# LFY1998/IPDM-PyTorch

Hardware: AMD Instinct MI355X
Metric: CT slices/s (full proj+img partial-diffusion sample) (higher is better)
Workload: dtype f32

## Files before the change

### include/ipdm_hip.h

```cpp
#ifndef IPDM_HIP_H
#define IPDM_HIP_H
#include <stddef.h>
#include <stdint.h>

#ifdef __cplusplus
extern "C" {
#endif

#define IPDM_OK 0
#define IPDM_ERR_INVALID (-1)
#define IPDM_ERR_HIP (-2)
#define IPDM_ERR_WORKSPACE (-3)
#define IPDM_ERR_UNSUPPORTED (-4)

const char *ipdm_last_error(void);
#define IPDM_ABI_VERSION 5
int ipdm_abi_version(void);

int ipdm_set_option(const char *name, int value);
int ipdm_get_option(const char *name, int *value);

typedef struct ipdm_fbp_geom {
    int32_t n_views, n_det, grid_n;
    double da, det_offset, dtheta_deg, source_origin, fov_half;
// ... 142 lines not shown
int ipdm_metrics_plan_destroy(ipdm_metrics_plan *plan);
size_t ipdm_metrics_workspace_bytes(const ipdm_metrics_plan *plan, int32_t B, uint32_t mask);
int ipdm_metrics(ipdm_metrics_plan *plan, const float *d_ref, int64_t ref_stride, const float *d_img, int32_t B,
                 uint32_t mask, double *d_out, void *d_ws, size_t ws_bytes, void *stream);
int64_t ipdm_metrics_table(const ipdm_metrics_plan *plan, int32_t which, void *host_out, int64_t cap_elems);

int ipdm_lowdose_noise(const float *d_proj, const float *d_z1, const float *d_z2, float *d_out, int32_t B,
                       int64_t n_per_slice, double factor, double n0, double ne, int32_t model, void *stream);
int ipdm_lowdose_noise_rng(const float *d_proj, float *d_out, int32_t B, int64_t n_per_slice, double factor, double n0,
                           double ne, int32_t model, uint64_t seed, int64_t slice_id0, int64_t draw0, void *stream);

#define IPDM_PROF_CLASSES 8
int ipdm_profile_begin(int32_t max_launches);
int ipdm_profile_begin_classes(int32_t max_launches, uint32_t class_mask);
int ipdm_profile_end(double *out_flops, double *out_ms, int64_t *out_launches, int32_t n_classes);
int ipdm_clock_probe(uint64_t *d_out, int32_t samples, int32_t period_us, void *stream);

int ipdm_bench_conv2d(int32_t B, int32_t C1, int32_t C2, int32_t H, int32_t W, int32_t Cout, int32_t ksize,
                      int32_t stride, int32_t act, int32_t with_res, int32_t iters, float *avg_ms);
int ipdm_bench_attention(int32_t B, int32_t heads, int32_t d, int32_t T, int32_t iters, float *avg_ms);
int32_t ipdm_conv_layout_code(int32_t Cout, int32_t ksize, int32_t stride);
int32_t ipdm_conv_kernel_code(int32_t B, int32_t Cout, int32_t Cin, int32_t ksize, int32_t stride, int32_t H, int32_t W);
int32_t ipdm_conv_kernel_code_stats(int32_t B, int32_t Cout, int32_t Cin, int32_t ksize, int32_t stride, int32_t H, int32_t W);
int32_t ipdm_attention_kernel_code(int32_t d);

#ifdef __cplusplus
}
#endif
#endif
```

### ipdm-pytorch_amd/_lib.py

```python
import ctypes as C
import os

_HERE = os.path.dirname(os.path.abspath(__file__))
LIB_PATH = os.environ.get("IPDM_LIB_PATH") or os.path.join(_HERE, "libipdm_hip.so")


class IpdmError(RuntimeError):
    pass


class FbpGeom(C.Structure):
    _fields_ = [("n_views", C.c_int32), ("n_det", C.c_int32), ("grid_n", C.c_int32),
                ("da", C.c_double), ("det_offset", C.c_double), ("dtheta_deg", C.c_double),
                ("source_origin", C.c_double), ("fov_half", C.c_double)]


class UnetCfg(C.Structure):
    _fields_ = [("in_channels", C.c_int32), ("model_channels", C.c_int32), ("out_channels", C.c_int32),
                ("num_res_blocks", C.c_int32), ("num_heads", C.c_int32), ("n_mult", C.c_int32),
                ("n_attn", C.c_int32), ("channel_mult", C.c_double * 16),
                ("attention_resolutions", C.c_int32 * 16)]


class ReverseArgs(C.Structure):
# ... 54 lines not shown
    "ipdm_ddpm_step_rng": (C.c_int, [_vp, _i32, _vp, _vp, _vp, _u64, _i64, _i64, _vp, _i32, _i32, _i32, _f64, _vp, _i32, _i32,
                                     _i32, _vp, _sz, _vp]),
    "ipdm_reverse_workspace_bytes": (_sz, [_vp, _i32, _i32, _i32]),
    "ipdm_reverse_pass": (C.c_int, [_vp, _vp, _vp, _vp, _vp, _i32, _i32, _vp, _i32, _i32, _i32, _i32, C.POINTER(ReverseArgs),
                                    _vp, _sz, _vp]),
    "ipdm_guided_reverse": (C.c_int, [_vp, _vp, _vp, _vp, _i32, _i32, _i32, C.POINTER(_i32), _i32, C.POINTER(ReverseArgs),
                                      C.POINTER(_i64), _vp, _sz, _vp]),
    "ipdm_op_conv2d": (C.c_int, [_vp, _i32, _vp, _i32, _i32, _i32, _i32, _i32, _i32, _vp, _vp, _i32, _i32, _i32,
                                 _i32, _i32, _vp, _vp, _vp, _vp, _vp]),
    "ipdm_op_conv_gn_conv": (C.c_int, [_vp, _i32, _i32, _i32, _i32, _vp, _vp, _i32, _i32, _i32, _vp, _i32, _vp, _vp, _i32, _vp, _vp,
                                       _i32, _vp, _vp, C.POINTER(_i32), _vp]),
    "ipdm_op_up_conv_chain": (C.c_int, [_vp, _i32, _i32, _i32, _i32, _vp, _vp, _i32, _vp, _i32, _i32, _vp, _vp, _i32, _vp, _vp,
                                        _i32, _i32, _vp, _vp, C.POINTER(_i32), _vp]),
    "ipdm_profile_begin": (C.c_int, [_i32]),
    "ipdm_profile_begin_classes": (C.c_int, [_i32, C.c_uint32]),
    "ipdm_clock_probe": (C.c_int, [_vp, _i32, _i32, _vp]),
    "ipdm_profile_end": (C.c_int, [C.POINTER(_f64 * PROF_CLASSES), C.POINTER(_f64 * PROF_CLASSES), C.POINTER(_i64 * PROF_CLASSES), _i32]),
    "ipdm_bench_conv2d": (C.c_int, [_i32] * 11 + [C.POINTER(_f32)]),
    "ipdm_bench_attention": (C.c_int, [_i32] * 5 + [C.POINTER(_f32)]),
    "ipdm_op_attention": (C.c_int, [_vp, _vp, _i32, _i32, _i32, _i32, _vp]),
    "ipdm_conv_layout_code": (_i32, [_i32, _i32, _i32]),
    "ipdm_conv_kernel_code": (_i32, [_i32, _i32, _i32, _i32, _i32, _i32, _i32]),
    "ipdm_conv_kernel_code_stats": (_i32, [_i32, _i32, _i32, _i32, _i32, _i32, _i32]),
    "ipdm_attention_kernel_code": (_i32, [_i32]),
    "ipdm_art_plan_create": (C.c_int, [_vp, _vp, _vp, C.POINTER(_vp)]),
    "ipdm_art_plan_destroy": (C.c_int, [_vp]),
    "ipdm_art_workspace_bytes": (C.c_size_t, [_vp, _i32]),
    "ipdm_art_reconstruct": (C.c_int, [_vp, _vp, _vp, _i32, _i32, _i32, _i32, _vp, C.c_size_t, _vp]),
    "ipdm_art_project": (C.c_int, [_vp, _vp, _vp, _i32, _vp, C.c_size_t, _vp]),
    "ipdm_metrics_plan_create": (C.c_int, [_i32, _i32, C.POINTER(_vp)]),
    "ipdm_metrics_plan_destroy": (C.c_int, [_vp]),
    "ipdm_metrics_workspace_bytes": (_sz, [_vp, _i32, C.c_uint32]),
    "ipdm_metrics": (C.c_int, [_vp, _vp, _i64, _vp, _i32, C.c_uint32, _vp, _vp, _sz, _vp]),
    "ipdm_metrics_table": (_i64, [_vp, _i32, _vp, _i64]),
    "ipdm_lowdose_noise": (C.c_int, [_vp, _vp, _vp, _vp, _i32, _i64, _f64, _f64, _f64, _i32, _vp]),
    "ipdm_lowdose_noise_rng": (C.c_int, [_vp, _vp, _i32, _i64, _f64, _f64, _f64, _i32, _u64, _i64, _i64, _vp]),
}

_lib = None


def lib():
    global _lib
    if _lib is None:
        if not os.path.isfile(LIB_PATH):
            raise IpdmError("%s not found: the HIP extension is mandatory (no CPU fallback). "
# ... 64 lines not shown
```

### ipdm-pytorch_amd/csrc/common.h

```cpp
#pragma once
#include <hip/hip_runtime.h>
#include <cstdarg>
#include <cstdio>
#include <cstring>
#include <string>
#include <vector>
#include "../../include/ipdm_hip.h"

namespace ipdm {

void set_error(const char *fmt, ...);

#define IPDM_HIP_CHECK(expr)                                                                   \
    do {                                                                                       \
        hipError_t e_ = (expr);                                                                \
        if (e_ != hipSuccess) {                                                                \
            ipdm::set_error("%s failed: %s (%s:%d)", #expr, hipGetErrorString(e_), __FILE__,  \
                            __LINE__);                                                         \
            return IPDM_ERR_HIP;                                                               \
        }                                                                                      \
    } while (0)

#define IPDM_REQUIRE(cond, ...)                   \
    do {                                          \
// ... 2 lines not shown
            return IPDM_ERR_INVALID;              \
        }                                         \
    } while (0)

#define IPDM_LAUNCH_CHECK() IPDM_HIP_CHECK(hipGetLastError())

static inline int cdiv(long a, long b) { return (int)((a + b - 1) / b); }
static inline size_t align_up(size_t v, size_t a) { return (v + a - 1) / a * a; }

enum Opt {
    OPT_CONV_NO_UP2,
    OPT_CONV_NO_WUP2,
    OPT_CONV_LEGACY, OPT_CONV1X1_LEGACY, OPT_CONVS2_LEGACY,
    OPT_CONV_NO_DIRECT, OPT_DIRECT_NO_PLANAR, OPT_DIRECT_MAX_CIN, OPT_DIRECT_NO_S2, OPT_DIRECT_NO_SKIP_FUSE,
    OPT_CONV_DBG, OPT_CONV_VEC4_STRICT, OPT_CONV_NO_SPLITK, OPT_CONV_NO_WINO, OPT_WINO_V1, OPT_WINO2_MIN_TILES, OPT_CONV1X1_NO_QUARTER, OPT_CONV_NO_PW, OPT_PW_ITEM, OPT_PW_FORCE,
    OPT_CONV_NM,
    OPT_GN_TWO_STAGE, OPT_GN_UNFUSED,
    OPT_UNET_TRANSPOSE,
    OPT_ATTN_NO_KVSPLIT, OPT_ATTN_LEGACY, OPT_ATTN_NO_ZSEQ,
    OPT_ART_PER_VIEW,
    OPT_CONV_BF16X3,
    OPT_ATTN_EXACT_F32,
    OPT_ATTN_NO_PRESPLIT,
    OPT_COUNT
};
int opt(Opt o);
bool opt_per_call(int o);
const char *opt_name(int o);
void opt_snapshot(int (&dst)[OPT_COUNT]);
int opt_changed_since(const int (&rec)[OPT_COUNT]);
std::vector<int> opt_per_call_values();

int ensure_dynamic_lds(const void *kernel, size_t bytes);
int device_cu_count();

int unet_io_channels(const ipdm_unet *net, int *cin, int *cout);

__device__ inline double wave_sum(double v)
{
#pragma unroll
    for (int o = 32; o > 0; o >>= 1) v += __shfl_down(v, o, 64);
    return v;
}
__device__ inline float wave_sum(float v)
{
#pragma unroll
// ... 12 lines not shown
```

### ipdm-pytorch_amd/csrc/common.hip

```cpp
#include <cctype>
#include <cstdlib>
#include <mutex>
#include <strings.h>
#include <set>
#include <utility>
#include "common.h"

namespace ipdm {
static thread_local char g_err[512] = "";
void set_error(const char *fmt, ...)
{
    va_list ap;
    va_start(ap, fmt);
    vsnprintf(g_err, sizeof(g_err), fmt, ap);
    va_end(ap);
}

namespace {
std::mutex g_attr_mu;
std::set<std::pair<const void *, int>> g_attr_done;
int g_cus[64];
}

namespace {
struct OptDef { const char *name; int def; bool per_call; int lo = 0, hi = 1; };
const OptDef g_opt_def[OPT_COUNT] = {
    {"conv_no_up2", 0, true},
    {"conv_no_wup2", 0, true},
    {"conv_legacy", 0, false}, {"conv1x1_legacy", 0, false}, {"convs2_legacy", 0, false},
    {"conv_no_direct", 0, false}, {"direct_no_planar", 0, false},
    {"direct_max_cin", 160, false, 0, 160},
    {"direct_no_s2", 0, false}, {"direct_no_skip_fuse", 0, true},
    {"conv_dbg", 0, true, 0, 0x3ff}, {"conv_vec4_strict", 0, false}, {"conv_no_splitk", 0, false},
    {"conv_no_wino", 0, true}, {"wino_v1", 0, true}, {"wino2_min_tiles", 192, true, 0, 1 << 24},
    {"conv1x1_no_quarter", 0, true}, {"conv_no_pw", 0, true}, {"pw_item", 0, true, 0, 2}, {"pw_force", 0, true}, {"conv_nm", 0, true, 0, 2},
    {"gn_two_stage", 0, true}, {"gn_unfused", 0, true},
    {"unet_transpose", -1, true, -1, 1},
    {"attn_no_kvsplit", 0, false}, {"attn_legacy", 0, false}, {"attn_no_zseq", 0, true},
    {"art_per_view", 0, true},
    {"conv_bf16x3", 0, true},
    {"attn_exact_f32", 0, true},
    {"attn_no_presplit", 0, true},
};
bool opt_value_ok(int i, int v)
{
    return v >= g_opt_def[i].lo && v <= g_opt_def[i].hi;
}
std::mutex g_opt_mu;
int g_opt_val[OPT_COUNT];
bool g_opt_init = false;

void opt_init_locked()
{
    if (g_opt_init) return;
    for (int i = 0; i < OPT_COUNT; ++i) {
        char env[64] = "IPDM_";
        size_t n = 5;
        for (const char *c = g_opt_def[i].name; *c && n + 1 < sizeof(env); ++c) env[n++] = (char)toupper((unsigned char)*c);
        env[n] = 0;
        const char *e = getenv(env);
        g_opt_val[i] = g_opt_def[i].def;
        if (e) {
            char *end = nullptr;
            const long v = strtol(e, &end, 10);
            const int want = (end != e) ? (int)v : 1;
// ... 93 lines not shown
```

### ipdm-pytorch_amd/csrc/conv_direct.hip

```cpp
#include <cstdlib>
#include <type_traits>
#include "common.h"
#include "unet_kernels.h"

using namespace ipdm;

typedef float f32x2 __attribute__((ext_vector_type(2)));
typedef float f32x4 __attribute__((ext_vector_type(4)));

namespace {

inline double direct_bytes(const ConvArgs &a)
{
    return 4.0 * a.B * ((double)(a.C1 + a.C2 + (a.sk_w ? a.sk_C1 + a.sk_C2 : 0)) * a.Hs * a.Ws + (double)a.Cout * a.Ho * a.Wo * (a.res ? 2 : 1));
}

inline bool direct_compute_bound(const ConvArgs &a) { return a.C1 + a.C2 >= 64; }
inline double direct_flops(const ConvArgs &a, int taps)
{
    return 2.0 * a.B * a.Ho * a.Wo * a.Cout * ((double)(a.C1 + a.C2) * taps + (a.sk_w ? a.sk_C1 + a.sk_C2 : 0));
}
inline int direct_class(const ConvArgs &a) { return direct_compute_bound(a) ? 6 : 4; }
inline double direct_work(const ConvArgs &a, int taps) { return direct_compute_bound(a) ? direct_flops(a, taps) : direct_bytes(a); }

// ... 12 lines not shown
    const int rest = t / gx;
    d.by = rest % gy;
    d.n = rest / gy;
    return d;
}
constexpr int DIN_P1 = 68;

#define IPDM_DPP_F(v, ctrl) __builtin_bit_cast(float, __builtin_amdgcn_update_dpp(0, __builtin_bit_cast(int, (v)), (ctrl), 0xf, 0xf, false))
__device__ inline float sum_lanes_row(float x)
{
    x += IPDM_DPP_F(x, 0x121);
    x += IPDM_DPP_F(x, 0x122);
    x += IPDM_DPP_F(x, 0x124);
    x += IPDM_DPP_F(x, 0x128);
    return x;
}
#undef IPDM_DPP_F

constexpr int DOOB = 0x7fffffff;
__device__ inline float dload(__amdgpu_buffer_rsrc_t r, int voff, int soff)
{
    return __builtin_bit_cast(float, __builtin_amdgcn_raw_buffer_load_b32(r, voff, soff, 0));
}

template <int CO>
__device__ inline void direct_epilogue(const ConvArgs &a, f32x2 (&acc)[4][CO / 2], int n, int ox0, int oy0, int tx, int ty, float *in_lds)
{
    const int tid = threadIdx.x;
    const int oy = oy0 + ty, ox = ox0 + tx * 4;
    const bool in_img = oy < a.Ho && ox < a.Wo;
    const size_t out_plane = (size_t)a.Ho * a.Wo;
    const bool vec = (a.Wo & 3) == 0;
    const bool full_tile = oy0 + DT_H <= a.Ho && ox0 + DT_W <= a.Wo;
    float *st = in_lds;
    if (a.stats) __syncthreads();
#pragma unroll
    for (int co = 0; co < CO; ++co) {
        if (co < a.Cout) {
            const float b = a.bias ? a.bias[co] : 0.0f;
            const size_t o = ((size_t)n * a.Cout + co) * out_plane + (size_t)oy * a.Wo + ox;
            f32x4 v = {acc[0][co / 2][co & 1] + b, acc[1][co / 2][co & 1] + b, acc[2][co / 2][co & 1] + b, acc[3][co / 2][co & 1] + b};
            if (in_img) {
                if (vec) {
                    if (a.res) v += *reinterpret_cast<const f32x4 *>(a.res + o);
                    *reinterpret_cast<f32x4 *>(a.out + o) = v;
                } else {
// ... 15 lines not shown
            }
        }
    }
    if (a.stats) {
        __syncthreads();
        const int j = tid & 15;
#pragma unroll
        for (int k = tid >> 4; k < 2 * CO; k += 16) {
            if ((k >> 1) < a.Cout) {
                const f32x4 *src = reinterpret_cast<const f32x4 *>(st + k * 256 + j * 16);
                const f32x4 p0 = src[0], p1 = src[1], p2 = src[2], p3 = src[3];
                float s = (((p0[0] + p0[1]) + (p0[2] + p0[3])) + ((p1[0] + p1[1]) + (p1[2] + p1[3]))) +
                          (((p2[0] + p2[1]) + (p2[2] + p2[3])) + ((p3[0] + p3[1]) + (p3[2] + p3[3])));
                s = sum_lanes_row(s);
                if (j == 0) {
                    const int row = (oy0 / DT_H) * gridDim.x + ox0 / DT_W;
                    a.stats[(((size_t)n * a.stats_rows + row) * a.Cout + (k >> 1)) * 2 + (k & 1)] = s;
                }
            }
        }
    }
}

template <int CO, int KS, int DKC, bool PLANAR, int STRIDE = 1, int SKIP = 0>
__global__ void __launch_bounds__(256, (STRIDE == 2 ? (CO <= 8 ? 4 : 3) : (CO <= 4 ? 6 : (CO <= 8 ? 5 : 3)))) conv_direct_kernel(ConvArgs a)
{
    static_assert(SKIP == 0 || (KS == 3 && STRIDE == 1 && !PLANAR), "conv_direct: the fused shortcut rides on a 3x3 stride-1 NCHW layer");
    constexpr int DIN_H = (DT_H - 1) * STRIDE + KS, DIN_W = (DT_W - 1) * STRIDE + KS, DIN_P = STRIDE == 1 ? DIN_P1 : 132;
    constexpr int DIN_CH = DIN_H * DIN_P, TAPS = KS * KS, PAD = KS / 2;
    static_assert(STRIDE == 1 || (KS == 3 && !PLANAR), "conv_direct: stride 2 is the 3x3 Downsample");
    __shared__ __attribute__((aligned(16))) float in_lds[DKC * DIN_CH];
    typedef const __attribute__((address_space(4))) float cfloat;
    cfloat *wk = (cfloat *)(unsigned long long)a.w;
    cfloat *gsc = (cfloat *)(unsigned long long)a.gn_scale, *gsh = (cfloat *)(unsigned long long)a.gn_shift;
    const int tid = threadIdx.x;
    const int tx = tid & 15, ty = tid >> 4;
    const DTile dt = direct_tile();
    const int n = dt.n;
    const int ox0 = dt.bx * DT_W, oy0 = dt.by * DT_H;
    const int Ctot = a.C1 + a.C2;
    const int src_plane = a.Hs * a.Ws;

    f32x2 acc[4][CO / 2];
#pragma unroll
    for (int p = 0; p < 4; ++p)
#pragma unroll
        for (int c = 0; c < CO / 2; ++c) acc[p][c] = f32x2{0.0f, 0.0f};

    constexpr int NSP = (DIN_H * DIN_W + 255) / 256;
    int sp_src[NSP], sp_srcp[NSP], sp_dst[NSP];
    bool sp_ok[NSP];
#pragma unroll
    for (int j = 0; j < NSP; ++j) {
        const int e = tid + j * 256;
        const int r = e / DIN_W, c = e % DIN_W;
        const int iy = oy0 * STRIDE - PAD + r, ix = ox0 * STRIDE - PAD + c;
        sp_ok[j] = e < DIN_H * DIN_W && iy >= 0 && iy < a.H && ix >= 0 && ix < a.W;
        int sy = min(max(iy, 0), a.H - 1), sx = min(max(ix, 0), a.W - 1);
        if (a.upsample) {
            sy = min((int)floorf((float)sy * a.scale_y), a.Hs - 1);
            sx = min((int)floorf((float)sx * a.scale_x), a.Ws - 1);
        }
        sp_src[j] = e < DIN_H * DIN_W ? (sy * a.Ws + sx) * 4 : DOOB;
        sp_srcp[j] = !(PLANAR || SKIP == 2) ? sp_src[j]
                   : (e < DIN_H * DIN_W ? ((((sy & 1) * 2 + (sx & 1)) * (a.Hs >> 1) + (sy >> 1)) * (a.Ws >> 1) + (sx >> 1)) * 4 : DOOB);
        sp_dst[j] = e < DIN_H * DIN_W ? r * DIN_P + c : -1;
    }
    const int plane_bytes = src_plane * 4;
    const __amdgpu_buffer_rsrc_t rsrc1 = __builtin_amdgcn_make_buffer_rsrc((void *)(a.x1 + (size_t)n * a.C1 * src_plane), 0, a.C1 * plane_bytes, 0x00020000);
    const __amdgpu_buffer_rsrc_t rsrc2 = __builtin_amdgcn_make_buffer_rsrc((void *)(a.x2 ? a.x2 + (size_t)n * a.C2 * src_plane : a.x1), 0, a.x2 ? a.C2 * plane_bytes : 0, 0x00020000);

    auto run_chunks = [&](auto sk_tag) __attribute__((always_inline)) {
    constexpr bool SK = decltype(sk_tag)::value;
    const int C1v = SK ? a.sk_C1 : a.C1, Ctotv = SK ? a.sk_C1 + a.sk_C2 : Ctot;
    const int actv = SK ? 0 : a.act;
    const __amdgpu_buffer_rsrc_t rsA = SK ? __builtin_amdgcn_make_buffer_rsrc((void *)(a.sk_x1 + (size_t)n * a.sk_C1 * src_plane), 0, a.sk_C1 * plane_bytes, 0x00020000) : rsrc1;
    const __amdgpu_buffer_rsrc_t rsB = SK ? __builtin_amdgcn_make_buffer_rsrc((void *)(a.sk_x2 ? a.sk_x2 + (size_t)n * a.sk_C2 * src_plane : a.sk_x1), 0,
                                                                               a.sk_x2 ? a.sk_C2 * plane_bytes : 0, 0x00020000) : rsrc2;
    constexpr bool PL = SK ? SKIP == 2 : PLANAR;
    cfloat *wkv = SK ? (cfloat *)(unsigned long long)a.sk_w : wk;
    const int cpadv = SK ? a.sk_cout_pad : a.cout_pad;
    for (int c0 = 0; c0 < Ctotv; c0 += DKC) {
        const int kc = min(DKC, Ctotv - c0);
        __syncthreads();
        float raw[DKC][NSP];
#pragma unroll
        for (int c = 0; c < DKC; ++c) {
            const int cg = min(c0 + c, Ctotv - 1);
            const bool from1 = cg < C1v;
            const __amdgpu_buffer_rsrc_t r = from1 ? rsA : rsB;
            const int so = (from1 ? cg : cg - C1v) * plane_bytes;
#pragma unroll
            for (int j = 0; j < NSP; ++j) raw[c][j] = dload(r, PL && from1 ? sp_srcp[j] : sp_src[j], so);
        }
#pragma unroll
        for (int c = 0; c < DKC; ++c) {
            if (c < kc) {
                float sc = 1.0f, sh = 0.0f;
                if (actv) { sc = gsc[(size_t)n * Ctot + c0 + c]; sh = gsh[(size_t)n * Ctot + c0 + c]; }
#pragma unroll
                for (int j = 0; j < NSP; ++j) {
                    float v = raw[c][j];
                    if (actv) {
                        v = v * sc + sh;
                        if (actv == 2) v = v * __builtin_amdgcn_rcpf(1.0f + __builtin_amdgcn_exp2f(-1.4426950408889634f * v));
                    }
                    if (sp_dst[j] >= 0) in_lds[c * DIN_CH + sp_dst[j]] = sp_ok[j] ? v : 0.0f;
                }
            }
        }
        __syncthreads();
        for (int c = 0; c < kc; ++c) {
            const float *ip = in_lds + c * DIN_CH + ty * STRIDE * DIN_P + tx * 4 * STRIDE;
#pragma unroll
            for (int ky = 0; ky < KS; ++ky) {
                if (SK && ky != 1) continue;
                const f32x4 lo = *reinterpret_cast<const f32x4 *>(ip + ky * DIN_P);
                f32x2 hi = {0.0f, 0.0f};
                if (KS > 1 && STRIDE == 1) hi = *reinterpret_cast<const f32x2 *>(ip + ky * DIN_P + 4);
                f32x4 mid = {0.0f, 0.0f, 0.0f, 0.0f};
                float last = 0.0f;
                if (STRIDE == 2) { mid = *reinterpret_cast<const f32x4 *>(ip + ky * DIN_P + 4); last = ip[ky * DIN_P + 8]; }
                const float iv[9] = {lo[0], lo[1], lo[2], lo[3], STRIDE == 1 ? hi[0] : mid[0], STRIDE == 1 ? hi[1] : mid[1], mid[2], mid[3], last};
#pragma unroll
                for (int kx = 0; kx < KS; ++kx) {
                    if (SK && kx != 1) continue;
                    cfloat *wp = wkv + (SK ? (size_t)(c0 + c) : (size_t)(c0 + c) * TAPS + ky * KS + kx) * cpadv;
                    f32x2 wv[CO / 2];
#pragma unroll
                    for (int q = 0; q < CO / 2; ++q) wv[q] = f32x2{wp[2 * q], wp[2 * q + 1]};
#pragma unroll
                    for (int p = 0; p < 4; ++p)
#pragma unroll
                        for (int q = 0; q < CO / 2; ++q) acc[p][q] += wv[q] * iv[p * STRIDE + kx];
                }
            }
        }
    }

    };
    run_chunks(std::false_type{});
    if (SKIP) run_chunks(std::true_type{});

    static_assert(2 * CO * 256 <= DKC * DIN_CH, "conv_direct: statistics staging does not fit the input tile area");
    direct_epilogue<CO>(a, acc, n, ox0, oy0, tx, ty, in_lds);
}

template <int CO, int DKC>
__global__ void __launch_bounds__(256, (CO <= 8 ? 5 : 3)) conv_direct_up2_kernel(ConvArgs a)
{
    constexpr int SH = DT_H / 2 + 2, SW = DT_W / 2 + 2, SP = 36, SCH = SH * SP;
    constexpr int LDS_FLOATS = (DKC * SCH > 2 * CO * 256) ? DKC * SCH : 2 * CO * 256;
    __shared__ __attribute__((aligned(16))) float in_lds[LDS_FLOATS];
    typedef const __attribute__((address_space(4))) float cfloat;
    cfloat *wk = (cfloat *)(unsigned long long)a.w_up2;
    const int tid = threadIdx.x, wave = tid >> 6, lane = tid & 63;
    const int tx = lane & 15;
    const int ty = (wave >> 1) * 8 + (lane >> 4) * 2 + (wave & 1);
    const int par_a = __builtin_amdgcn_readfirstlane(wave & 1);
    const DTile dt = direct_tile();
    const int n = dt.n;
    const int ox0 = dt.bx * DT_W, oy0 = dt.by * DT_H;
    const int sx0 = (ox0 >> 1) - 1, sy0 = (oy0 >> 1) - 1;
    const int Cin = a.C1, src_plane = a.Hs * a.Ws, plane_bytes = src_plane * 4;
    const int cin_pad = (Cin + 7) / 8 * 8;
// ... 57 lines not shown
        }
    }
    direct_epilogue<CO>(a, acc, n, ox0, oy0, tx, ty, in_lds);
}

template <int CO>
int launch_direct_s2(const ConvArgs &a, hipStream_t st)
{
    dim3 grid(cdiv(a.Wo, DT_W), cdiv(a.Ho, DT_H), a.B);
    const bool prof = prof_enabled();
    if (prof) prof_before(direct_class(a), st);
    hipLaunchKernelGGL((conv_direct_kernel<CO, 3, 2, false, 2>), grid, dim3(256), 0, st, a);
    if (prof) prof_after(direct_class(a), direct_work(a, 9), st);
    IPDM_LAUNCH_CHECK();
    return IPDM_OK;
}

template <int CO, int KS>
int launch_direct(const ConvArgs &a, hipStream_t st)
{
    dim3 grid(cdiv(a.Wo, DT_W), cdiv(a.Ho, DT_H), a.B);
    const bool prof = prof_enabled();
    if (prof) prof_before(direct_class(a), st);
    if constexpr (KS == 3 && CO >= 8) {
        if (a.sk_w) {
            if (a.sk_planar) hipLaunchKernelGGL((conv_direct_kernel<CO, KS, (CO <= 8 ? 4 : 8), false, 1, 2>), grid, dim3(256), 0, st, a);
            else hipLaunchKernelGGL((conv_direct_kernel<CO, KS, (CO <= 8 ? 4 : 8), false, 1, 1>), grid, dim3(256), 0, st, a);
            if (prof) prof_after(direct_class(a), direct_work(a, KS * KS), st);
            IPDM_LAUNCH_CHECK();
            return IPDM_OK;
        }
    }
    if (a.x1_planar) hipLaunchKernelGGL((conv_direct_kernel<CO, KS, (CO <= 8 ? 4 : 8), true>), grid, dim3(256), 0, st, a);
    else hipLaunchKernelGGL((conv_direct_kernel<CO, KS, (CO <= 8 ? 4 : 8), false>), grid, dim3(256), 0, st, a);
    if (prof) prof_after(direct_class(a), direct_work(a, KS * KS), st);
    IPDM_LAUNCH_CHECK();
    return IPDM_OK;
}

}

namespace ipdm {

bool conv_direct_eligible(const ConvArgs &a)
{
    const int max_cin = opt(OPT_DIRECT_MAX_CIN);
    const int cin = a.C1 + a.C2;
    const bool no_s2 = opt(OPT_DIRECT_NO_S2) != 0;
    if (a.stride == 2)
        return !no_s2 && a.ksize == 3 && a.Cout <= 16 && cin <= 32 && !a.upsample && !a.x1_planar && a.w_interleave == 0 && a.cout_pad >= 16;
    return (a.ksize == 3 || a.ksize == 1) && a.stride == 1 && a.Cout <= 16 && (cin <= max_cin || (a.Cout <= 4 && cin <= 128)) && a.w_interleave == 0 &&
           a.cout_pad >= 16;
}

bool conv_direct_up2_eligible(const ConvArgs &a)
{
    const bool off = opt(OPT_CONV_NO_UP2) != 0;
    return !off && a.w_up2 && a.w_interleave == 0 && a.ksize == 3 && a.stride == 1 && a.C2 == 0 && a.act == 0 && !a.res &&
           !a.x1_planar && a.H == 2 * a.Hs && a.W == 2 * a.Ws && a.Ho == a.H && a.Wo == a.W && a.Cout > 4 && a.Cout <= 16 &&
           a.C1 <= 64 && a.cout_pad >= 16;
}

int conv_direct_stats_rows(const ConvArgs &a) { return cdiv(a.Wo, DT_W) * cdiv(a.Ho, DT_H); }

bool conv_direct_skip_ok(const ConvArgs &a)
{
    if (opt(OPT_CONV_NO_DIRECT) || opt(OPT_DIRECT_NO_SKIP_FUSE)) return false;
    return conv_direct_eligible(a) && a.ksize == 3 && a.stride == 1 && !a.upsample && !a.x1_planar && !a.C2 && !a.res && a.Cout > 4 && a.Cout <= 16 &&
           a.sk_C1 > 0 && a.sk_C1 + a.sk_C2 <= opt(OPT_DIRECT_MAX_CIN) && a.sk_cout_pad >= 16 && !conv_direct_up2_eligible(a);
}

int conv2d_direct_launch(const ConvArgs &a, hipStream_t st)
{
    IPDM_REQUIRE(conv_direct_eligible(a), "conv2d_direct: layer not eligible");
    IPDM_REQUIRE(!a.stats || a.stats_rows == conv_direct_stats_rows(a), "conv2d: statistics rows %d != %d", a.stats_rows,
                 conv_direct_stats_rows(a));
    IPDM_REQUIRE(!a.x1_planar || (!a.upsample && !(a.Hs & 1) && !(a.Ws & 1)), "conv2d: parity-planar input of odd size %dx%d", a.Hs, a.Ws);
    IPDM_REQUIRE((long)a.C1 * a.Hs * a.Ws < (1L << 29) && (long)(a.C2 + 1) * a.Hs * a.Ws < (1L << 29),
                 "conv2d: per-sample tensor exceeds the 2 GiB buffer-addressing range");
    IPDM_REQUIRE(!a.sk_w || conv_direct_skip_ok(a), "conv2d: this layer cannot carry a fused shortcut");
    IPDM_REQUIRE(!a.sk_w || ((long)a.sk_C1 * a.Hs * a.Ws < (1L << 29) && (long)(a.sk_C2 + 1) * a.Hs * a.Ws < (1L << 29)),
                 "conv2d: the fused shortcut's source exceeds the 2 GiB buffer-addressing range");
    IPDM_REQUIRE(!a.sk_w || !a.sk_planar || (!(a.Hs & 1) && !(a.Ws & 1)), "conv2d: parity-planar shortcut source of odd size %dx%d", a.Hs, a.Ws);
// ... 27 lines not shown
```

### ipdm-pytorch_amd/csrc/unet.hip

```cpp
#include <algorithm>
#include <cmath>
#include <cstdlib>
#include <map>
#include <string>
#include <tuple>
#include <vector>
#include "unet_kernels.h"

using namespace ipdm;

namespace {

__global__ void __launch_bounds__(256) temb_kernel(const float *__restrict__ freqs, int mc, float t,
                                                   const float *__restrict__ w0, const float *__restrict__ b0,
                                                   const float *__restrict__ w2, const float *__restrict__ b2,
                                                   float *__restrict__ tmp, float *__restrict__ silu_emb)
{
    extern __shared__ float sm[];
    float *e0 = sm;
    float *h1 = sm + mc;
    const int half = mc / 2, ted = 4 * mc;
    for (int i = threadIdx.x; i < mc; i += 256) {
        float v = 0.0f;
        if (i < half) v = cosf(t * freqs[i]);
// ... 354 lines not shown
namespace {

#ifndef IPDM_UNET_TRACE
#define IPDM_UNET_TRACE 0
#endif
#if IPDM_UNET_TRACE
__global__ void trace_sum_kernel(const unsigned *p, size_t n, unsigned long long *slot)
{
    unsigned long long s = 0;
    for (size_t i = (size_t)blockIdx.x * blockDim.x + threadIdx.x; i < n; i += (size_t)gridDim.x * blockDim.x) s += (unsigned long long)p[i] * (i % 1021 + 1);
    atomicAdd(slot, s);
}
std::vector<std::string> g_trace_desc;
unsigned long long *g_trace_slots = nullptr;
struct TraceRec { size_t off, n; int B, C, H, W; size_t off_x1 = 0, off_sc = 0, off_sh = 0; int C1 = 0, code = 0; const float *w = nullptr; };
std::vector<TraceRec> g_trace_rec;
char *g_trace_pool = nullptr;
size_t g_trace_used = 0;
const size_t g_trace_pool_bytes = (size_t)48 << 30;
int trace_code(const ConvArgs &a) { return conv_plan(a, a.stats != nullptr, a.split_ws != nullptr).code; }
void trace_conv(const ConvArgs &a, size_t n, hipStream_t st)
{
    char desc[256];
    snprintf(desc, sizeof(desc), "code %2d  %3d+%-3d -> %3d @%4dx%-4d s%d act %d res %d planar %d stats %d", trace_code(a), a.C1, a.C2, a.Cout, a.Ho, a.Wo,
             a.stride, a.act, a.res ? 1 : 0, a.x1_planar, a.stats ? a.stats_rows : 0);
#if IPDM_UNET_TRACE == 1
    std::vector<unsigned> h(n);
    (void)hipStreamSynchronize(st);
    (void)hipMemcpy(h.data(), a.out, n * 4, hipMemcpyDeviceToHost);
    unsigned long long sum = 0;
    for (size_t i = 0; i < n; ++i) sum += (unsigned long long)h[i] * (i % 1021 + 1);
    fprintf(stderr, "TRACE %4zu %s  %016llx\n", g_trace_desc.size(), desc, sum);
    g_trace_desc.push_back(desc);
#elif IPDM_UNET_TRACE == 3
    if (!g_trace_pool) { (void)hipMalloc((void **)&g_trace_pool, g_trace_pool_bytes); }
    if (g_trace_used + n * 4 <= g_trace_pool_bytes) {
        (void)hipMemcpyAsync(g_trace_pool + g_trace_used, a.out, n * 4, hipMemcpyDeviceToDevice, st);
        TraceRec rec{g_trace_used, n, a.B, a.Cout, a.Ho, a.Wo};
        g_trace_used += (n * 4 + 255) / 256 * 256;
        rec.code = trace_code(a);
        const size_t nx = (size_t)a.B * a.C1 * a.Hs * a.Ws * 4, ng = (size_t)a.B * (a.C1 + a.C2) * 4;
        if (rec.code == 12 && a.C2 == 0 && a.act && g_trace_used + nx + 2 * ng + 1024 <= g_trace_pool_bytes) {
            rec.C1 = a.C1; rec.w = a.w_wino;
            rec.off_x1 = g_trace_used; (void)hipMemcpyAsync(g_trace_pool + g_trace_used, a.x1, nx, hipMemcpyDeviceToDevice, st); g_trace_used += (nx + 255) / 256 * 256;
            rec.off_sc = g_trace_used; (void)hipMemcpyAsync(g_trace_pool + g_trace_used, a.gn_scale, ng, hipMemcpyDeviceToDevice, st); g_trace_used += (ng + 255) / 256 * 256;
            rec.off_sh = g_trace_used; (void)hipMemcpyAsync(g_trace_pool + g_trace_used, a.gn_shift, ng, hipMemcpyDeviceToDevice, st); g_trace_used += (ng + 255) / 256 * 256;
        }
        g_trace_rec.push_back(rec);
// ... 973 lines not shown
    const int pad = ksize / 2;
    ConvArgs a;
    a.x1 = &dummy; a.x2 = nullptr; a.C1 = Cin; a.C2 = 0; a.B = B; a.Hs = H; a.Ws = W; a.H = H; a.W = W; a.upsample = 0;
    a.scale_y = a.scale_x = 1.f; a.w = &dummy; a.bias = nullptr; a.Cout = Cout; a.ksize = ksize; a.stride = stride;
    a.w_interleave = conv_weight_interleave(Cout, ksize, stride);
    const int group = a.w_interleave ? 32 * a.w_interleave : 64;
    a.cout_pad = (Cout + group - 1) / group * group;
    a.Ho = (H + 2 * pad - ksize) / stride + 1; a.Wo = (W + 2 * pad - ksize) / stride + 1;
    a.act = 0; a.gn_scale = a.gn_shift = nullptr; a.res = nullptr; a.out = &dummy;
    a.tiles_x = a.tiles_y = a.co_tiles = 0;
    a.w_wino = conv_wino_shape_ok(Cout, Cin, ksize, stride, a.w_interleave) ? &dummy : nullptr;
    return conv_plan(a, with_stats, true).code;
}

extern "C" int32_t ipdm_conv_kernel_code(int32_t B, int32_t Cout, int32_t Cin, int32_t ksize, int32_t stride, int32_t H, int32_t W)
{
    return conv_kernel_code_impl(B, Cout, Cin, ksize, stride, H, W, false);
}
extern "C" int32_t ipdm_conv_kernel_code_stats(int32_t B, int32_t Cout, int32_t Cin, int32_t ksize, int32_t stride, int32_t H, int32_t W)
{
    return conv_kernel_code_impl(B, Cout, Cin, ksize, stride, H, W, true);
}

extern "C" int ipdm_bench_attention(int32_t B, int32_t heads, int32_t d, int32_t T, int32_t iters, float *avg_ms)
{
    IPDM_REQUIRE(avg_ms && iters > 0, "bench_attention: bad argument");
    float *d_qkv, *d_out;
    IPDM_HIP_CHECK(hipMalloc((void **)&d_qkv, (size_t)B * heads * 3 * d * T * 4));
    IPDM_HIP_CHECK(hipMalloc((void **)&d_out, (size_t)B * heads * d * T * 4));
    ipdm_randn(d_qkv, B, (int64_t)heads * 3 * d * T, 9, 0, 0, nullptr);
    int rc = 0;
    float *d_scr = nullptr;
    if (attention_scratch_floats(B, heads, d, T)) IPDM_HIP_CHECK(hipMalloc((void **)&d_scr, attention_scratch_floats(B, heads, d, T) * 4));
    float *d_pl = nullptr;
    if (attention_planes_floats(B, heads, d, T)) IPDM_HIP_CHECK(hipMalloc((void **)&d_pl, attention_planes_floats(B, heads, d, T) * 4));
    for (int i = 0; i < 2 && !rc; ++i) rc = attention_launch(d_qkv, d_out, B, heads, d, T, nullptr, d_scr, d_pl);
    hipEvent_t e0, e1;
    IPDM_HIP_CHECK(hipEventCreate(&e0));
    IPDM_HIP_CHECK(hipEventCreate(&e1));
    IPDM_HIP_CHECK(hipEventRecord(e0, nullptr));
    for (int i = 0; i < iters && !rc; ++i) rc = attention_launch(d_qkv, d_out, B, heads, d, T, nullptr, d_scr, d_pl);
    IPDM_HIP_CHECK(hipEventRecord(e1, nullptr));
    IPDM_HIP_CHECK(hipEventSynchronize(e1));
    float ms = 0;
    IPDM_HIP_CHECK(hipEventElapsedTime(&ms, e0, e1));
    *avg_ms = ms / iters;
// ... 77 lines not shown
```

### ipdm-pytorch_amd/csrc/unet_kernels.h

```cpp
#pragma once
#include <vector>
#include "common.h"

namespace ipdm {

struct GnTileSrc { const float *stats = nullptr; int rows = 0, C = 0; };
struct GnTileArgs {
    GnTileSrc src[2];
    int nsrc = 1, B = 0;
    long HW = 0;
    int groups = 0;
    const float *gamma = nullptr, *beta = nullptr;
    float eps = 1e-5f;
    double *partials = nullptr;
    float *scale = nullptr, *shift = nullptr;
};

struct ConvArgs {
    const float *x1, *x2;
    int C1, C2, B;
    int Hs, Ws;
    int H, W;
    int upsample;
    float scale_y, scale_x;
// ... 18 lines not shown
    const float *sk_x1 = nullptr, *sk_x2 = nullptr, *sk_w = nullptr;
    int sk_C1 = 0, sk_C2 = 0, sk_cout_pad = 0, sk_planar = 0;
    int x1_planar = 0;
    int up2 = 0;
    int dbg = 0;
    unsigned long long *dbg_buf = nullptr;
};

struct ConvPlan {
    int code = 0;
    int ksplit = 1;
    size_t split_ws_bytes = 0;
    int stats_rows = 0;
    bool up2 = false;
    bool out_planar = false;
};
ConvPlan conv_plan(const ConvArgs &a, bool want_stats, bool may_split);
bool conv_planar_ok(const ConvArgs &a);
int conv2d_launch(const ConvArgs &a, hipStream_t st);

int conv2d_igemm_launch(const ConvArgs &a, hipStream_t st);
bool conv_direct_eligible(const ConvArgs &a);
bool conv_direct_up2_eligible(const ConvArgs &a);
bool conv_direct_skip_ok(const ConvArgs &a);
int conv2d_direct_launch(const ConvArgs &a, hipStream_t st);
bool conv_nm_eligible(const ConvArgs &a);
int conv2d_nm_launch(const ConvArgs &a, hipStream_t st);
int conv2d_ws_launch(const ConvArgs &a, hipStream_t st);
int conv_ws_split(const ConvArgs &a);
bool conv_ws_planar_ok(const ConvArgs &a);
int conv2d_splitk_launch(const ConvArgs &a, const ConvPlan &p, hipStream_t st);
bool conv_up2_eligible(const ConvArgs &a);
int conv2d_up2_launch(const ConvArgs &a, hipStream_t st);
bool conv_wup2_shape_ok(int Cout, int Cin);
bool conv_wup2_eligible(const ConvArgs &a);
int conv2d_wup2_launch(const ConvArgs &orig, hipStream_t st, int prof_cls);
bool conv_wino_shape_ok(int Cout, int Cin, int ks, int stride, int interleave);
bool conv_wino_eligible(const ConvArgs &a);
int conv2d_wino_launch(const ConvArgs &a, int code, hipStream_t st);
int conv_wino_split(const ConvArgs &a);
bool conv_wino2_eligible(const ConvArgs &a);
bool conv_wino3_eligible(const ConvArgs &a);
int conv2d_wino2_launch(const ConvArgs &prepared, hipStream_t st);
int conv2d_wino3_launch(const ConvArgs &prepared, hipStream_t st);
bool conv_pw_eligible(const ConvArgs &a, bool stats);
int conv2d_pw_launch(const ConvArgs &a, hipStream_t st);
// ... 50 lines not shown
```

Before: 2.176.

## Add vectorized fast input staging for interior tiles in direct conv

Adds a fast staging path to the direct convolution kernel. For workgroups whose input window lies fully inside the image, it loads the tile with 128-bit buffer loads plus separate halo and extra-row loads. The GN/SiLU transform is specialised per activation and applied while writing into LDS. The LDS tile is shifted by a 3-float offset so the vector stores stay aligned, which means the compute loop now rebuilds each window from unaligned pieces. This aims to cut per-element index math and scalar global loads during staging, at the cost of extra template instantiations, register pressure and a slightly costlier LDS read pattern.

```diff
diff --git a/include/ipdm_hip.h b/include/ipdm_hip.h
--- a/include/ipdm_hip.h
+++ b/include/ipdm_hip.h
@@ -188,6 +188,7 @@
 int32_t ipdm_conv_layout_code(int32_t Cout, int32_t ksize, int32_t stride);
 int32_t ipdm_conv_kernel_code(int32_t B, int32_t Cout, int32_t Cin, int32_t ksize, int32_t stride, int32_t H, int32_t W);
 int32_t ipdm_conv_kernel_code_stats(int32_t B, int32_t Cout, int32_t Cin, int32_t ksize, int32_t stride, int32_t H, int32_t W);
+int32_t ipdm_conv_direct_stage(int32_t Cout, int32_t Cin, int32_t ksize, int32_t stride, int32_t H, int32_t W, int32_t upsample, int32_t planar);
 int32_t ipdm_attention_kernel_code(int32_t d);
 
 #ifdef __cplusplus
diff --git a/ipdm-pytorch_amd/_lib.py b/ipdm-pytorch_amd/_lib.py
--- a/ipdm-pytorch_amd/_lib.py
+++ b/ipdm-pytorch_amd/_lib.py
@@ -100,6 +100,7 @@
     "ipdm_conv_layout_code": (_i32, [_i32, _i32, _i32]),
     "ipdm_conv_kernel_code": (_i32, [_i32, _i32, _i32, _i32, _i32, _i32, _i32]),
     "ipdm_conv_kernel_code_stats": (_i32, [_i32, _i32, _i32, _i32, _i32, _i32, _i32]),
+    "ipdm_conv_direct_stage": (_i32, [_i32] * 8),
     "ipdm_attention_kernel_code": (_i32, [_i32]),
     "ipdm_art_plan_create": (C.c_int, [_vp, _vp, _vp, C.POINTER(_vp)]),
     "ipdm_art_plan_destroy": (C.c_int, [_vp]),
diff --git a/ipdm-pytorch_amd/csrc/common.h b/ipdm-pytorch_amd/csrc/common.h
--- a/ipdm-pytorch_amd/csrc/common.h
+++ b/ipdm-pytorch_amd/csrc/common.h
@@ -48,6 +48,7 @@
     OPT_CONV_BF16X3,
     OPT_ATTN_EXACT_F32,
     OPT_ATTN_NO_PRESPLIT,
+    OPT_DIRECT_OLD_STAGE,
     OPT_COUNT
 };
 int opt(Opt o);
diff --git a/ipdm-pytorch_amd/csrc/common.hip b/ipdm-pytorch_amd/csrc/common.hip
--- a/ipdm-pytorch_amd/csrc/common.hip
+++ b/ipdm-pytorch_amd/csrc/common.hip
@@ -41,6 +41,7 @@
     {"conv_bf16x3", 0, true},
     {"attn_exact_f32", 0, true},
     {"attn_no_presplit", 0, true},
+    {"direct_old_stage", 0, true},
 };
 bool opt_value_ok(int i, int v)
 {
diff --git a/ipdm-pytorch_amd/csrc/conv_direct.hip b/ipdm-pytorch_amd/csrc/conv_direct.hip
--- a/ipdm-pytorch_amd/csrc/conv_direct.hip
+++ b/ipdm-pytorch_amd/csrc/conv_direct.hip
@@ -1,3 +1,4 @@
+#include <algorithm>
 #include <cstdlib>
 #include <type_traits>
 #include "common.h"
@@ -58,6 +59,20 @@
 {
     return __builtin_bit_cast(float, __builtin_amdgcn_raw_buffer_load_b32(r, voff, soff, 0));
 }
+__device__ inline f32x4 dload4(__amdgpu_buffer_rsrc_t r, int voff, int soff)
+{
+    return __builtin_bit_cast(f32x4, __builtin_amdgcn_raw_buffer_load_b128(r, voff, soff, 0));
+}
+
+template <int ACT>
+__device__ inline float stage_act(float v, float sc, float sh)
+{
+    if (ACT) {
+        v = fmaf(v, sc, sh);
+        if (ACT == 2) v = v * __builtin_amdgcn_rcpf(1.0f + __builtin_amdgcn_exp2f(-1.4426950408889634f * v));
+    }
+    return v;
+}
 
 template <int CO>
 __device__ inline void direct_epilogue(const ConvArgs &a, f32x2 (&acc)[4][CO / 2], int n, int ox0, int oy0, int tx, int ty, float *in_lds)
@@ -119,14 +134,16 @@
     }
 }
 
-template <int CO, int KS, int DKC, bool PLANAR, int STRIDE = 1, int SKIP = 0>
+template <int CO, int KS, int DKC, bool PLANAR, int STRIDE = 1, int SKIP = 0, int STG = 0>
 __global__ void __launch_bounds__(256, (STRIDE == 2 ? (CO <= 8 ? 4 : 3) : (CO <= 4 ? 6 : (CO <= 8 ? 5 : 3)))) conv_direct_kernel(ConvArgs a)
 {
     static_assert(SKIP == 0 || (KS == 3 && STRIDE == 1 && !PLANAR), "conv_direct: the fused shortcut rides on a 3x3 stride-1 NCHW layer");
+    static_assert(STG == 0 || (STRIDE == 1 && !PLANAR), "conv_direct: the fast staging path reads a stride-1 NCHW window");
+    constexpr int LOFF = (STG && KS == 3) ? 3 : 0;
     constexpr int DIN_H = (DT_H - 1) * STRIDE + KS, DIN_W = (DT_W - 1) * STRIDE + KS, DIN_P = STRIDE == 1 ? DIN_P1 : 132;
     constexpr int DIN_CH = DIN_H * DIN_P, TAPS = KS * KS, PAD = KS / 2;
     static_assert(STRIDE == 1 || (KS == 3 && !PLANAR), "conv_direct: stride 2 is the 3x3 Downsample");
-    __shared__ __attribute__((aligned(16))) float in_lds[DKC * DIN_CH];
+    __shared__ __attribute__((aligned(16))) float in_lds[DKC * DIN_CH + (LOFF ? 4 : 0)];
     typedef const __attribute__((address_space(4))) float cfloat;
     cfloat *wk = (cfloat *)(unsigned long long)a.w;
     cfloat *gsc = (cfloat *)(unsigned long long)a.gn_scale, *gsh = (cfloat *)(unsigned long long)a.gn_shift;
@@ -147,6 +164,8 @@
     constexpr int NSP = (DIN_H * DIN_W + 255) / 256;
     int sp_src[NSP], sp_srcp[NSP], sp_dst[NSP];
     bool sp_ok[NSP];
+    const bool fast_wg = STG && oy0 - PAD >= 0 && oy0 + DT_H + PAD <= a.H && ox0 - PAD >= 0 && ox0 + DT_W + PAD <= a.W;
+    if (!fast_wg || SKIP == 2) {
 #pragma unroll
     for (int j = 0; j < NSP; ++j) {
         const int e = tid + j * 256;
@@ -161,14 +180,16 @@
         sp_src[j] = e < DIN_H * DIN_W ? (sy * a.Ws + sx) * 4 : DOOB;
         sp_srcp[j] = !(PLANAR || SKIP == 2) ? sp_src[j]
                    : (e < DIN_H * DIN_W ? ((((sy & 1) * 2 + (sx & 1)) * (a.Hs >> 1) + (sy >> 1)) * (a.Ws >> 1) + (sx >> 1)) * 4 : DOOB);
-        sp_dst[j] = e < DIN_H * DIN_W ? r * DIN_P + c : -1;
+        sp_dst[j] = e < DIN_H * DIN_W ? r * DIN_P + c + LOFF : -1;
+    }
     }
     const int plane_bytes = src_plane * 4;
     const __amdgpu_buffer_rsrc_t rsrc1 = __builtin_amdgcn_make_buffer_rsrc((void *)(a.x1 + (size_t)n * a.C1 * src_plane), 0, a.C1 * plane_bytes, 0x00020000);
     const __amdgpu_buffer_rsrc_t rsrc2 = __builtin_amdgcn_make_buffer_rsrc((void *)(a.x2 ? a.x2 + (size_t)n * a.C2 * src_plane : a.x1), 0, a.x2 ? a.C2 * plane_bytes : 0, 0x00020000);
 
-    auto run_chunks = [&](auto sk_tag) __attribute__((always_inline)) {
+    auto run_chunks = [&](auto sk_tag, auto fast_tag) __attribute__((always_inline)) {
     constexpr bool SK = decltype(sk_tag)::value;
+    constexpr bool FAST = decltype(fast_tag)::value;
     const int C1v = SK ? a.sk_C1 : a.C1, Ctotv = SK ? a.sk_C1 + a.sk_C2 : Ctot;
     const int actv = SK ? 0 : a.act;
     const __amdgpu_buffer_rsrc_t rsA = SK ? __builtin_amdgcn_make_buffer_rsrc((void *)(a.sk_x1 + (size_t)n * a.sk_C1 * src_plane), 0, a.sk_C1 * plane_bytes, 0x00020000) : rsrc1;
@@ -180,6 +201,70 @@
     for (int c0 = 0; c0 < Ctotv; c0 += DKC) {
         const int kc = min(DKC, Ctotv - c0);
         __syncthreads();
+        if constexpr (FAST) {
+        constexpr int RSH = SK ? PAD : 0;
+        constexpr int NX = (KS == 3 && !SK) ? DKC / 4 : 0;
+        const int wv = __builtin_amdgcn_readfirstlane(tid >> 6), lane = tid & 63;
+        const int f_main = ((oy0 - PAD + ty + RSH) * a.Ws + ox0 + tx * 4) * 4;
+        float *l_main = in_lds + (ty + RSH) * DIN_P + LOFF + PAD + tx * 4;
+        const int xrow = DT_H + ((lane >> 4) & 1), hl = lane >= 36 ? lane - 36 : lane, hrow = hl >> 1, hcol = (hl & 1) * (DT_W + 1);
+        const int f_ext = ((oy0 - PAD + xrow) * a.Ws + ox0 + tx * 4) * 4, f_halo = ((oy0 - PAD + hrow) * a.Ws + ox0 - PAD + hcol) * 4;
+        float *l_ext = in_lds + xrow * DIN_P + LOFF + PAD + tx * 4, *l_halo = in_lds + hrow * DIN_P + LOFF + hcol;
+        f32x4 rawm[DKC], rawx[NX ? NX : 1];
+        float rawh[NX ? NX : 1];
+        int cx[NX ? NX : 1];
+#pragma unroll
+        for (int c = 0; c < DKC; ++c) {
+            const int cg = min(c0 + c, Ctotv - 1);
+            const bool from1 = cg < C1v;
+            rawm[c] = dload4(from1 ? rsA : rsB, f_main, (from1 ? cg : cg - C1v) * plane_bytes);
+        }
+        auto transform = [&](auto act_tag) __attribute__((always_inline)) {
+            constexpr int ACT = decltype(act_tag)::value;
+#pragma unroll
+            for (int c = 0; c < DKC / 2; ++c) {
+                if (c < kc) {
+                    float sc = 1.0f, sh = 0.0f;
+                    if (ACT) { sc = gsc[(size_t)n * Ctot + c0 + c]; sh = gsh[(size_t)n * Ctot + c0 + c]; }
+                    const f32x4 v = rawm[c];
+                    *reinterpret_cast<f32x4 *>(l_main + c * DIN_CH) =
+                        f32x4{stage_act<ACT>(v[0], sc, sh), stage_act<ACT>(v[1], sc, sh), stage_act<ACT>(v[2], sc, sh), stage_act<ACT>(v[3], sc, sh)};
+                }
+            }
+#pragma unroll
+            for (int h = 0; h < NX; ++h) {
+                cx[h] = min(c0 + wv + 4 * h, Ctotv - 1);
+                const bool from1 = cx[h] < C1v;
+                const __amdgpu_buffer_rsrc_t r = from1 ? rsA : rsB;
+                const int so = (from1 ? cx[h] : cx[h] - C1v) * plane_bytes;
+                rawx[h] = dload4(r, f_ext, so);
+                rawh[h] = dload(r, f_halo, so);
+            }
+#pragma unroll
+            for (int c = DKC / 2; c < DKC; ++c) {
+                if (c < kc) {
+                    float sc = 1.0f, sh = 0.0f;
+                    if (ACT) { sc = gsc[(size_t)n * Ctot + c0 + c]; sh = gsh[(size_t)n * Ctot + c0 + c]; }
+                    const f32x4 v = rawm[c];
+                    *reinterpret_cast<f32x4 *>(l_main + c * DIN_CH) =
+                        f32x4{stage_act<ACT>(v[0], sc, sh), stage_act<ACT>(v[1], sc, sh), stage_act<ACT>(v[2], sc, sh), stage_act<ACT>(v[3], sc, sh)};
+                }
+            }
+#pragma unroll
+            for (int h = 0; h < NX; ++h) {
+                float sc = 1.0f, sh = 0.0f;
+                if (ACT) { sc = gsc[(size_t)n * Ctot + cx[h]]; sh = gsh[(size_t)n * Ctot + cx[h]]; }
+                const f32x4 v = rawx[h];
+                const int lc = (wv + 4 * h) * DIN_CH;
+                *reinterpret_cast<f32x4 *>(l_ext + lc) =
+                    f32x4{stage_act<ACT>(v[0], sc, sh), stage_act<ACT>(v[1], sc, sh), stage_act<ACT>(v[2], sc, sh), stage_act<ACT>(v[3], sc, sh)};
+                l_halo[lc] = stage_act<ACT>(rawh[h], sc, sh);
+            }
+        };
+        if (actv == 0) transform(std::integral_constant<int, 0>{});
+        else if (actv == 1) transform(std::integral_constant<int, 1>{});
+        else transform(std::integral_constant<int, 2>{});
+        } else {
         float raw[DKC][NSP];
 #pragma unroll
         for (int c = 0; c < DKC; ++c) {
@@ -206,15 +291,23 @@
                 }
             }
         }
+        }
         __syncthreads();
         for (int c = 0; c < kc; ++c) {
             const float *ip = in_lds + c * DIN_CH + ty * STRIDE * DIN_P + tx * 4 * STRIDE;
 #pragma unroll
             for (int ky = 0; ky < KS; ++ky) {
                 if (SK && ky != 1) continue;
-                const f32x4 lo = *reinterpret_cast<const f32x4 *>(ip + ky * DIN_P);
+                f32x4 lo;
                 f32x2 hi = {0.0f, 0.0f};
-                if (KS > 1 && STRIDE == 1) hi = *reinterpret_cast<const f32x2 *>(ip + ky * DIN_P + 4);
+                if constexpr (LOFF != 0) {
+                    const f32x4 run = *reinterpret_cast<const f32x4 *>(ip + ky * DIN_P + 4);
+                    lo = f32x4{ip[ky * DIN_P + 3], run[0], run[1], run[2]};
+                    hi = f32x2{run[3], ip[ky * DIN_P + 8]};
+                } else {
+                    lo = *reinterpret_cast<const f32x4 *>(ip + ky * DIN_P);
+                    if (KS > 1 && STRIDE == 1) hi = *reinterpret_cast<const f32x2 *>(ip + ky * DIN_P + 4);
+                }
                 f32x4 mid = {0.0f, 0.0f, 0.0f, 0.0f};
                 float last = 0.0f;
                 if (STRIDE == 2) { mid = *reinterpret_cast<const f32x4 *>(ip + ky * DIN_P + 4); last = ip[ky * DIN_P + 8]; }
@@ -236,8 +329,18 @@
     }
 
     };
-    run_chunks(std::false_type{});
-    if (SKIP) run_chunks(std::true_type{});
+    if constexpr (STG != 0) {
+        if (fast_wg) {
+            run_chunks(std::false_type{}, std::true_type{});
+            if (SKIP) run_chunks(std::true_type{}, std::integral_constant<bool, SKIP == 1>{});
+        } else {
+            run_chunks(std::false_type{}, std::false_type{});
+            if (SKIP) run_chunks(std::true_type{}, std::false_type{});
+        }
+    } else {
+        run_chunks(std::false_type{}, std::false_type{});
+        if (SKIP) run_chunks(std::true_type{}, std::false_type{});
+    }
 
     static_assert(2 * CO * 256 <= DKC * DIN_CH, "conv_direct: statistics staging does not fit the input tile area");
     direct_epilogue<CO>(a, acc, n, ox0, oy0, tx, ty, in_lds);
@@ -341,9 +444,12 @@
     dim3 grid(cdiv(a.Wo, DT_W), cdiv(a.Ho, DT_H), a.B);
     const bool prof = prof_enabled();
     if (prof) prof_before(direct_class(a), st);
+    const bool stg = conv_direct_stage(a) > 0;
     if constexpr (KS == 3 && CO >= 8) {
         if (a.sk_w) {
-            if (a.sk_planar) hipLaunchKernelGGL((conv_direct_kernel<CO, KS, (CO <= 8 ? 4 : 8), false, 1, 2>), grid, dim3(256), 0, st, a);
+            if (a.sk_planar && stg) hipLaunchKernelGGL((conv_direct_kernel<CO, KS, (CO <= 8 ? 4 : 8), false, 1, 2, 1>), grid, dim3(256), 0, st, a);
+            else if (a.sk_planar) hipLaunchKernelGGL((conv_direct_kernel<CO, KS, (CO <= 8 ? 4 : 8), false, 1, 2>), grid, dim3(256), 0, st, a);
+            else if (stg) hipLaunchKernelGGL((conv_direct_kernel<CO, KS, (CO <= 8 ? 4 : 8), false, 1, 1, 1>), grid, dim3(256), 0, st, a);
             else hipLaunchKernelGGL((conv_direct_kernel<CO, KS, (CO <= 8 ? 4 : 8), false, 1, 1>), grid, dim3(256), 0, st, a);
             if (prof) prof_after(direct_class(a), direct_work(a, KS * KS), st);
             IPDM_LAUNCH_CHECK();
@@ -351,6 +457,7 @@
         }
     }
     if (a.x1_planar) hipLaunchKernelGGL((conv_direct_kernel<CO, KS, (CO <= 8 ? 4 : 8), true>), grid, dim3(256), 0, st, a);
+    else if (stg) hipLaunchKernelGGL((conv_direct_kernel<CO, KS, (CO <= 8 ? 4 : 8), false, 1, 0, 1>), grid, dim3(256), 0, st, a);
     else hipLaunchKernelGGL((conv_direct_kernel<CO, KS, (CO <= 8 ? 4 : 8), false>), grid, dim3(256), 0, st, a);
     if (prof) prof_after(direct_class(a), direct_work(a, KS * KS), st);
     IPDM_LAUNCH_CHECK();
@@ -378,6 +485,21 @@
     return !off && a.w_up2 && a.w_interleave == 0 && a.ksize == 3 && a.stride == 1 && a.C2 == 0 && a.act == 0 && !a.res &&
            !a.x1_planar && a.H == 2 * a.Hs && a.W == 2 * a.Ws && a.Ho == a.H && a.Wo == a.W && a.Cout > 4 && a.Cout <= 16 &&
            a.C1 <= 64 && a.cout_pad >= 16;
+}
+
+int conv_direct_stage(const ConvArgs &a)
+{
+    if (opt(OPT_DIRECT_OLD_STAGE)) return 0;
+    if (a.stride != 1 || (a.ksize != 3 && a.ksize != 1) || a.upsample || a.x1_planar || a.H != a.Hs || a.W != a.Ws) return 0;
+    if (conv_direct_up2_eligible(a)) return 0;
+    if (a.W & 3) return 0;
+    if (a.C1 + a.C2 < (a.Cout <= 4 ? 8 : 4)) return 0;
+    auto aligned = [](const float *p) { return ((unsigned long long)p & 15) == 0; };
+    if (!aligned(a.x1) || (a.C2 && !aligned(a.x2))) return 0;
+    if (a.sk_w && (!aligned(a.sk_x1) || (a.sk_C2 && !aligned(a.sk_x2)))) return 0;
+    const int pad = a.ksize / 2;
+    auto interior = [pad](int L, int T) { return L - T - pad < 0 ? 0 : std::max(0, (L - T - pad) / T - (pad ? 1 : 0) + 1); };
+    return interior(a.W, DT_W) * interior(a.H, DT_H);
 }
 
 int conv_direct_stats_rows(const ConvArgs &a) { return cdiv(a.Wo, DT_W) * cdiv(a.Ho, DT_H); }
diff --git a/ipdm-pytorch_amd/csrc/unet.hip b/ipdm-pytorch_amd/csrc/unet.hip
--- a/ipdm-pytorch_amd/csrc/unet.hip
+++ b/ipdm-pytorch_amd/csrc/unet.hip
@@ -400,8 +400,8 @@
 void trace_conv(const ConvArgs &a, size_t n, hipStream_t st)
 {
     char desc[256];
-    snprintf(desc, sizeof(desc), "code %2d  %3d+%-3d -> %3d @%4dx%-4d s%d act %d res %d planar %d stats %d", trace_code(a), a.C1, a.C2, a.Cout, a.Ho, a.Wo,
-             a.stride, a.act, a.res ? 1 : 0, a.x1_planar, a.stats ? a.stats_rows : 0);
+    snprintf(desc, sizeof(desc), "code %2d  %3d+%-3d -> %3d @%4dx%-4d s%d act %d res %d planar %d stats %d stage %d", trace_code(a), a.C1, a.C2, a.Cout, a.Ho, a.Wo,
+             a.stride, a.act, a.res ? 1 : 0, a.x1_planar, a.stats ? a.stats_rows : 0, trace_code(a) == 5 ? conv_direct_stage(a) : 0);
 #if IPDM_UNET_TRACE == 1
     std::vector<unsigned> h(n);
     (void)hipStreamSynchronize(st);
@@ -1421,6 +1421,25 @@
     return conv_kernel_code_impl(B, Cout, Cin, ksize, stride, H, W, true);
 }
 
+extern "C" int32_t ipdm_conv_direct_stage(int32_t Cout, int32_t Cin, int32_t ksize, int32_t stride, int32_t H, int32_t W, int32_t upsample, int32_t planar)
+{
+    if (Cout <= 0 || Cin <= 0 || H <= 0 || W <= 0 || (ksize != 1 && ksize != 3) || stride < 1 || stride > 2) return -1;
+    const int pad = ksize / 2;
+    ConvArgs a;
+    a.x1 = nullptr; a.x2 = nullptr; a.C1 = Cin; a.C2 = 0; a.B = 1; a.H = H; a.W = W; a.upsample = upsample ? 1 : 0;
+    a.Hs = upsample ? H / 2 : H; a.Ws = upsample ? W / 2 : W;
+    a.scale_y = a.scale_x = upsample ? 0.5f : 1.f; a.w = nullptr; a.bias = nullptr; a.Cout = Cout; a.ksize = ksize; a.stride = stride;
+    a.w_interleave = conv_weight_interleave(Cout, ksize, stride);
+    const int group = a.w_interleave ? 32 * a.w_interleave : 64;
+    a.cout_pad = (Cout + group - 1) / group * group;
+    a.Ho = (H + 2 * pad - ksize) / stride + 1; a.Wo = (W + 2 * pad - ksize) / stride + 1;
+    a.act = 0; a.gn_scale = a.gn_shift = nullptr; a.res = nullptr; a.out = nullptr;
+    a.tiles_x = a.tiles_y = a.co_tiles = 0;
+    a.x1_planar = planar ? 1 : 0;
+    if (a.w_interleave || opt(OPT_CONV_NO_DIRECT) || !conv_direct_eligible(a)) return -1;
+    return conv_direct_stage(a);
+}
+
 extern "C" int ipdm_bench_attention(int32_t B, int32_t heads, int32_t d, int32_t T, int32_t iters, float *avg_ms)
 {
     IPDM_REQUIRE(avg_ms && iters > 0, "bench_attention: bad argument");
diff --git a/ipdm-pytorch_amd/csrc/unet_kernels.h b/ipdm-pytorch_amd/csrc/unet_kernels.h
--- a/ipdm-pytorch_amd/csrc/unet_kernels.h
+++ b/ipdm-pytorch_amd/csrc/unet_kernels.h
@@ -64,6 +64,7 @@
 int conv2d_igemm_launch(const ConvArgs &a, hipStream_t st);
 bool conv_direct_eligible(const ConvArgs &a);
 bool conv_direct_up2_eligible(const ConvArgs &a);
+int conv_direct_stage(const ConvArgs &a);
 bool conv_direct_skip_ok(const ConvArgs &a);
 int conv2d_direct_launch(const ConvArgs &a, hipStream_t st);
 bool conv_nm_eligible(const ConvArgs &a);
```

After: 2.176, median of 6. Within noise of the previous version (+0.0%).
